# agwi-lab/renderformer

Measured on NVIDIA B200. Metric: frames/sec (512^2, 4096 tris), higher is better.
Workload: dtype bf16

## Files before the change

include/rfb200.h:

```cpp
#ifndef RFB200_H_
#define RFB200_H_

#include <stdint.h>

#ifdef __cplusplus
extern "C" {
#endif

typedef void* rfb_stream_t;

enum {
  RFB_OK = 0,
  RFB_ERR_ARG = -1,
  RFB_ERR_ALIGN = -2,
  RFB_ERR_DRIVER = -3,
  RFB_ERR_TMAP = -4,
  RFB_ERR_LAUNCH = -5
};

enum { RFB_F32 = 0, RFB_BF16 = 1, RFB_F16 = 2 };

int rfb_version(void);
long long rfb_launch_count(void);

// ... 38 lines not shown
  float norm_eps;
  float* out_rscale;
  float* out_sumsq;
  int out_sumsq_ld;
  void* out16;
  int out16_dtype;
  long long ld16;
  const float* col_mul;
  const int* aux_row_map;
  void* vt_out;
  int vt_dtype;
  int vt_split;
  int vt_rows_per_batch;
  long long vt_ld;
  long long vt_batch_stride;
} rfb_gemm_args;

int rfb_gemm(const rfb_gemm_args* a, rfb_stream_t stream);

typedef struct {
  int B, H, Nq, Nk;
  const void* Q;
  long long ldq, q_batch_stride;
  const void* K;
  long long ldk, k_batch_stride;
  const void* Vt;
  long long ldvt, vt_batch_stride;
  void* O;
  long long ldo, o_batch_stride;
  const uint32_t* key_mask_bits;
// ... 79 lines not shown
```

renderformer_b200/csrc/gemm.cu:

```cuda
#include <stdlib.h>

#include <atomic>

#include "host_util.h"
#include "ptx.cuh"

namespace rfb {

std::atomic<long long> g_launch_count{0};

struct GemmKParams {
  int M, N, K;
  int num_m_tiles, num_n_tiles, num_kb;
  int a_mode;
  int H, Wd, Cin, tw, th, tiles_x, tiles_y, kb_per_tap;
  uint32_t idesc;
  int epi;
  const float* bias;
  const void* res1;
  const void* res2;
  int res_dtype;
  long long ldres;
  void* out;
  int out_dtype;
// ... 731 lines not shown
      if (cudaFuncGetAttributes(&fa, gemm_tc_kernel<BN, EK>) != cudaSuccess) return RFB_ERR_LAUNCH;
      if (128 * kRegsGemmWg0 + 256 * kRegsGemmEpi > kGemmThreadsWG * fa.numRegs) {
        fprintf(stderr, "rfb: gemm_tc_kernel<RESID> compiled with %d registers/thread; setmaxnreg split does not fit\n",
                fa.numRegs);
        return RFB_ERR_LAUNCH;
      }
    }
    attr_set = true;
  }
  constexpr int threads = ek_resid(EK) ? kGemmThreadsWG : kGemmThreads;
  gemm_tc_kernel<BN, EK><<<grid, threads, Cfg::kSmemBytes, stream>>>(tmA, tmB, p);
  g_launch_count++;
  return check_launch("gemm_tc_kernel");
}

constexpr int kHaloPitch = 18;
constexpr uint32_t kHaloBytes = kHaloPitch * kHaloPitch * 128;
constexpr uint32_t kHaloStride = 42 * 1024;

template <int BN>
struct HaloCfg {
  static constexpr uint32_t kBBytes = BN * kBK * 2;
  static constexpr int kStages = (BN == 128) ? 6 : 8;
  static constexpr uint32_t kTmemCols = (4 * BN < 32) ? 32 : 4 * BN;
  static constexpr uint32_t kSmemBytes = 2 * kHaloStride + kStages * kBBytes + 1024 + 256 + kEpiStageBytes;
};

template <int BN, int EK>
__global__ void __launch_bounds__(kGemmThreads, 1)
    conv_halo_kernel(const __grid_constant__ CUtensorMap tmA, const __grid_constant__ CUtensorMap tmB,
                     const GemmKParams p) {
  using Cfg = HaloCfg<BN>;
  constexpr int STAGES = Cfg::kStages;
  constexpr uint32_t B_BYTES = Cfg::kBBytes;

  extern __shared__ uint8_t smem_raw[];
  const uint32_t raw_addr = smem_u32(smem_raw);
  uint8_t* smem = smem_raw + ((1024u - (raw_addr & 1023u)) & 1023u);
  uint8_t* sH = smem;
  uint8_t* sB = smem + 2 * kHaloStride;
  uint64_t* bfull = reinterpret_cast<uint64_t*>(sB + STAGES * B_BYTES);
  uint64_t* bempty = bfull + STAGES;
  uint64_t* hfull = bempty + STAGES;
  uint64_t* hempty = hfull + 2;
  uint64_t* tfull = hempty + 2;
  uint64_t* tempty = tfull + 2;
  uint32_t* tmem_slot = reinterpret_cast<uint32_t*>(tempty + 2);
  float* epi_stage = reinterpret_cast<float*>(reinterpret_cast<uint8_t*>(bfull) + 256);

  const int warp = threadIdx.x >> 5;
  const int lane = threadIdx.x & 31;

  if (threadIdx.x == 0) {
    for (int i = 0; i < STAGES; ++i) mbar_init(&bfull[i], 1), mbar_init(&bempty[i], 1);
    for (int i = 0; i < 2; ++i) {
// ... 11 lines not shown
  tc_fence_before();
  __syncthreads();
  tc_fence_after();
  const uint32_t tmem_base = *tmem_slot;

  const int per_img = p.tiles_x * p.tiles_y;
  const int total = p.num_m_tiles;
  const int ncb = p.kb_per_tap;

  if (warp == 0) {
    if (lane == 0) {
      int stage = 0, hb = 0;
      uint32_t phase = 0, hphase = 0;
      for (int tile = blockIdx.x; tile < total; tile += gridDim.x) {
        const int bi = tile / per_img, rr = tile % per_img;
        const int y0 = (rr / p.tiles_x) * 16, x0 = (rr % p.tiles_x) * 16;
        for (int cb = 0; cb < ncb; ++cb) {
          mbar_wait(&hempty[hb], hphase ^ 1);
          mbar_expect_tx(&hfull[hb], kHaloBytes);
          tma_load_4d(sH + hb * kHaloStride, &tmA, &hfull[hb], cb * kBK, x0 - 1, y0 - 1, bi);
          if (++hb == 2) hb = 0, hphase ^= 1;
          for (int tap = 0; tap < 9; ++tap) {
            mbar_wait(&bempty[stage], phase ^ 1);
            mbar_expect_tx(&bfull[stage], B_BYTES);
            tma_load_2d(sB + stage * B_BYTES, &tmB, &bfull[stage], tap * p.Cin + cb * kBK, 0);
            if (++stage == STAGES) stage = 0, phase ^= 1;
          }
        }
      }
    }
  } else if (warp == 1) {
    if (lane == 0) {
      int stage = 0, hb = 0, it = 0;
      uint32_t phase = 0, hphase = 0;
      for (int tile = blockIdx.x; tile < total; tile += gridDim.x, ++it) {
        const int as = it & 1;
        mbar_wait(&tempty[as], ((it >> 1) & 1) ^ 1);
        tc_fence_after();
        const uint32_t d0 = tmem_base + as * 2 * BN;
        for (int cb = 0; cb < ncb; ++cb) {
          mbar_wait(&hfull[hb], hphase);
          tc_fence_after();
          const uint32_t halo = smem_u32(sH + hb * kHaloStride);
          for (int tap = 0; tap < 9; ++tap) {
            mbar_wait(&bfull[stage], phase);
            tc_fence_after();
            const uint64_t bd = umma_desc_sw128(smem_u32(sB + stage * B_BYTES));
            const uint32_t a0 = halo + ((tap / 3) * kHaloPitch + tap % 3) * 128;
#pragma unroll
            for (int t = 0; t < 2; ++t) {
              uint64_t ad = static_cast<uint64_t>(((a0 + t * 8 * 128) >> 4) & 0x3fff);
              ad |= static_cast<uint64_t>((kHaloPitch * 128) >> 4) << 32;
              ad |= static_cast<uint64_t>(1) << 46;
              ad |= static_cast<uint64_t>(2) << 61;
#pragma unroll
              for (int k = 0; k < kBK / 16; ++k)
                umma_f16(d0 + t * BN, ad + 2 * k, bd + 2 * k, p.idesc, (cb | tap | k) != 0);
            }
            umma_commit(&bempty[stage]);
            if (++stage == STAGES) stage = 0, phase ^= 1;
          }
          umma_commit(&hempty[hb]);
          if (++hb == 2) hb = 0, hphase ^= 1;
        }
        umma_commit(&tfull[as]);
      }
    }
  } else {
    const int q = warp & 3;
    const int r = q * 32 + lane;
    int it = 0;
    for (int tile = blockIdx.x; tile < total; tile += gridDim.x, ++it) {
      const int as = it & 1;
      const uint32_t aph = (it >> 1) & 1;
      const int bi = tile / per_img, rr = tile % per_img;
      const int y = (rr / p.tiles_x) * 16 + (r >> 3);
      float* my_stage = epi_stage + (warp - 2) * 32 * 32;
      constexpr int NCH = BN / 32;
      constexpr int HALF = (NCH + 1) / 2;
      const int c_begin = ((warp - 2) >> 2) * HALF;
      const int c_end = (c_begin + HALF < NCH) ? c_begin + HALF : NCH;
#pragma unroll 1
      for (int t = 0; t < 2; ++t) {
        const int x = (rr % p.tiles_x) * 16 + t * 8 + (r & 7);
        const bool valid = (y < p.H) && (x < p.Wd);
        const long long orow = (static_cast<long long>(bi) * p.H + y) * p.Wd + x;
        const int orow_mine = valid ? static_cast<int>(orow) : -1;
        const uint32_t taddr0 = tmem_base + (static_cast<uint32_t>(q * 32) << 16) + as * 2 * BN + t * BN;
        if (p.epi == RFB_EPI_STORE) {
          epilogue_generic_coalesced<EK>(p, my_stage, lane, taddr0, 0, c_begin, c_end, orow_mine, orow_mine, 1.0f,
                                         &tfull[as], aph);
        } else {
// ... 11 lines not shown
      }
      tc_fence_before();
      __syncwarp();
      if (lane == 0) mbar_arrive(&tempty[as]);
    }
  }

  tc_fence_before();
  __syncthreads();
  if (warp == 1) {
    tc_fence_after();
    tmem_dealloc(tmem_base, Cfg::kTmemCols);
  }
}

template <int BN, int EK = EK_GENERIC>
static int launch_conv_halo(const CUtensorMap& tmA, const CUtensorMap& tmB, const GemmKParams& p, int grid,
                            cudaStream_t stream) {
  using Cfg = HaloCfg<BN>;
  static PerDeviceFlag attr_flags;
  bool& attr_set = attr_flags.get();
  if (!attr_set) {
    if (cudaFuncSetAttribute(conv_halo_kernel<BN, EK>, cudaFuncAttributeMaxDynamicSharedMemorySize,
                             Cfg::kSmemBytes) != cudaSuccess)
      return RFB_ERR_LAUNCH;
    attr_set = true;
  }
  conv_halo_kernel<BN, EK><<<grid, kGemmThreads, Cfg::kSmemBytes, stream>>>(tmA, tmB, p);
  g_launch_count++;
  return check_launch("conv_halo_kernel");
}

}

using namespace rfb;

extern "C" int rfb_gemm(const rfb_gemm_args* a, rfb_stream_t stream_) {
  cudaStream_t stream = static_cast<cudaStream_t>(stream_);
  if (!a || !a->A || !a->W || a->M <= 0 || a->N <= 0 || a->K <= 0) return RFB_ERR_ARG;
  if (a->dtype != RFB_BF16 && a->dtype != RFB_F16) return RFB_ERR_ARG;

  GemmKParams p{};
  p.M = a->M, p.N = a->N, p.K = a->K;
// ... 7 lines not shown
  p.in_sumsq_parts = a->in_sumsq_parts > 0 ? a->in_sumsq_parts : 1;
  p.in_rscale = a->in_rscale, p.scale_dim = a->scale_dim, p.out_rscale = a->out_rscale;
  p.inv_norm_dim = a->norm_dim > 0 ? 1.0f / (float)a->norm_dim : 0.f;
  p.norm_eps = a->norm_eps;
  p.out_sumsq = a->out_sumsq, p.out_sumsq_ld = a->out_sumsq_ld;
  p.out16 = a->out16, p.out16_dtype = a->out16_dtype, p.ld16 = a->ld16;
  p.col_mul = a->col_mul, p.aux_row_map = a->aux_row_map;
  p.vt_out = a->vt_out, p.vt_dtype = a->vt_dtype, p.vt_split = a->vt_split;
  p.vt_rows_per_batch = a->vt_rows_per_batch, p.vt_ld = a->vt_ld, p.vt_batch_stride = a->vt_batch_stride;
  if (a->vt_out) {
    if (a->a_mode != RFB_A_LINEAR || a->epi != RFB_EPI_STORE || a->row_map || a->vt_split <= 0 || a->vt_split >= a->N ||
        a->vt_split % 256 || (a->vt_dtype != RFB_BF16 && a->vt_dtype != RFB_F16) || a->vt_ld < 1 ||
        (a->in_rscale && a->scale_dim == 1))
      return RFB_ERR_ARG;
  }
  const bool fused_any = a->in_sumsq || a->in_rscale || a->out_rscale || a->out_sumsq || a->out16 || a->col_mul;
  if (a->in_sumsq && (a->norm_dim <= 0 || a->in_rscale || p.in_sumsq_parts > p.in_sumsq_ld)) return RFB_ERR_ARG;
  if (a->in_rscale && a->scale_dim != 0 && a->scale_dim != 1) return RFB_ERR_ARG;
  if (a->out_rscale && !a->in_sumsq) return RFB_ERR_ARG;
  const bool epi_final = a->epi == RFB_EPI_FINAL || a->epi == RFB_EPI_FINAL_RAW;
  if (fused_any && epi_final) return RFB_ERR_ARG;
  if (a->epi == RFB_EPI_SWIGLU && (a->out_rscale || a->out_sumsq || a->out16 || a->col_mul ||
                                   (a->in_rscale && a->scale_dim != 0)))
    return RFB_ERR_ARG;
  if (a->out16 && (a->ld16 % 8 || (a->out16_dtype != RFB_BF16 && a->out16_dtype != RFB_F16))) return RFB_ERR_ARG;
  if (a->out16 && a->N % 8) return RFB_ERR_ARG;
  const int n_plain = a->vt_out ? a->vt_split : a->N;
  if (a->out_sumsq && (n_plain % 128 || a->out_sumsq_ld < n_plain / 128)) return RFB_ERR_ARG;
  if (a->res2 && (a->res_dtype == RFB_F32 || !a->res1)) return RFB_ERR_ARG;

  const bool resid_kind = a->epi == RFB_EPI_STORE && a->a_mode == RFB_A_LINEAR && a->N % 256 == 0 && a->out16 &&
                          a->out_sumsq && !a->bias && !a->res2 && !a->out_act && !a->vt_out && !a->col_mul &&
                          !(a->in_rscale && a->scale_dim == 1) && a->out && a->out_dtype == RFB_F32 && a->res1 &&
                          a->res_dtype == RFB_F32;
  const int sms = num_sms();
  const long long m_tiles_lin = (a->M + kBM - 1) / kBM;
  int bn = a->bn_override;
  if (a->vt_out) {
    if (bn != 0 && bn != 256) return RFB_ERR_ARG;
    bn = 256;
  }
  if (a->out_sumsq) {
// ... 18 lines not shown
  }
  if (bn != 32 && bn != 64 && bn != 128 && bn != 256) return RFB_ERR_ARG;

  if (a->epi == RFB_EPI_STORE) {
    p.n_store = (n_plain + 7) & ~7;
    if (p.n_store > a->ldo) return RFB_ERR_ARG;
    if ((a->bias || a->res1 || a->res2) && (a->N % 8) != 0) return RFB_ERR_ARG;
    if (!a->out && !a->out_act && !a->out16) return RFB_ERR_ARG;
    const int align = (a->out_dtype == RFB_F32) ? 4 : 8;
    if (a->ldo % align) return RFB_ERR_ALIGN;
    if ((a->res1 || a->res2) && a->ldres % ((a->res_dtype == RFB_F32) ? 4 : 8)) return RFB_ERR_ALIGN;
  } else if (a->epi == RFB_EPI_SWIGLU) {
    if (a->N % 32 || !a->out || a->out_dtype == RFB_F32 || a->ldo % 8) return RFB_ERR_ARG;
    p.n_store = a->N;
  } else if (epi_final) {
    if (a->N != 32 || !a->out || !a->bias || !a->w2 || !a->b2) return RFB_ERR_ARG;
    bn = 32;
    p.n_store = 32;
  } else {
    return RFB_ERR_ARG;
  }

  CUtensorMap tmA, tmB;
  int rc;
  if (a->a_mode == RFB_A_LINEAR) {
    uint64_t dims[2] = {(uint64_t)a->K, (uint64_t)a->M};
    uint64_t strides[1] = {(uint64_t)a->lda * 2};
    uint32_t box[2] = {(uint32_t)kBK, (uint32_t)kBM};
    if ((rc = make_tmap_16b(&tmA, a->dtype, a->A, 2, dims, strides, box)) != RFB_OK) return rc;
    p.num_m_tiles = (a->M + kBM - 1) / kBM;
    p.num_kb = (a->K + kBK - 1) / kBK;
  } else if (a->a_mode == RFB_A_CONV3X3) {
    if (a->B <= 0 || a->H <= 0 || a->Wd <= 0 || a->Cin <= 0 || a->K != 9 * a->Cin ||
        a->M != a->B * a->H * a->Wd || a->row_map)
      return RFB_ERR_ARG;
    {
      static int halo_on = -1;
      if (halo_on < 0) {
        const char* e = getenv("RFB_CONV_HALO");
        halo_on = (e && e[0] == '0') ? 0 : 1;
      }
      const int stx = (a->Wd + 15) / 16, sty = (a->H + 15) / 16;
      const long long n_super = (long long)a->B * stx * sty;
      if (halo_on && a->Cin % 64 == 0 && a->N == bn && (bn == 128 || bn == 64 || bn == 32) && n_super >= 96 &&
          !fused_any && !a->vt_out && !p.direct_store) {
        p.H = a->H, p.Wd = a->Wd, p.Cin = a->Cin;
        p.tw = 8, p.th = 16, p.tiles_x = stx, p.tiles_y = sty, p.kb_per_tap = a->Cin / kBK;
        p.num_m_tiles = (int)n_super, p.num_n_tiles = 1, p.num_kb = 9 * p.kb_per_tap;
        uint64_t dims[4] = {(uint64_t)a->Cin, (uint64_t)a->Wd, (uint64_t)a->H, (uint64_t)a->B};
        uint64_t strides[3] = {(uint64_t)a->Cin * 2, (uint64_t)a->Wd * a->Cin * 2, (uint64_t)a->H * a->Wd * a->Cin * 2};
        uint32_t box[4] = {(uint32_t)kBK, (uint32_t)kHaloPitch, (uint32_t)kHaloPitch, 1};
        if ((rc = make_tmap_16b(&tmA, a->dtype, a->A, 4, dims, strides, box)) != RFB_OK) return rc;
        uint64_t wd[2] = {(uint64_t)a->K, (uint64_t)a->N};
        uint64_t ws[1] = {(uint64_t)a->ldw * 2};
        uint32_t wb[2] = {(uint32_t)kBK, (uint32_t)bn};
        if ((rc = make_tmap_16b(&tmB, a->dtype, a->W, 2, wd, ws, wb)) != RFB_OK) return rc;
        p.idesc = umma_idesc_f16(a->dtype == RFB_BF16 ? 1u : 0u, kBM, bn);
        const int cap = a->max_ctas > 0 ? a->max_ctas : num_sms();
        const int grid = (int)(n_super < cap ? n_super : cap);
        if (bn == 64) return launch_conv_halo<64>(tmA, tmB, p, grid, stream);
        if (bn == 32) return launch_conv_halo<32>(tmA, tmB, p, grid, stream);
        if (a->epi == RFB_EPI_STORE && a->dtype == RFB_F16 && a->out_dtype == RFB_F16 &&
            (!a->res1 || a->res_dtype == RFB_F16)) {
          const int cm = (a->out ? CF_OUT : 0) | (a->out_act ? CF_ACT : 0) | (a->bias ? CF_BIAS : 0) |
                         (a->res1 ? CF_RES1 : 0) | (a->res2 ? CF_RES2 : 0);
          switch (cm) {
// ... 55 lines not shown
  if (bn == 128 && a->out_sumsq) {
    if (p.direct_store) return RFB_ERR_ARG;
    return a->out16_dtype == RFB_F16 ? launch_gemm<128, EK_RESID_H>(tmA, tmB, p, grid, stream)
                                     : launch_gemm<128, EK_RESID>(tmA, tmB, p, grid, stream);
  }
  if (bn == 256 && a->N % 256 == 0 && a->epi == RFB_EPI_STORE && !p.direct_store && a->out16 &&
      a->out_sumsq && !a->bias && !a->res2 && !a->out_act && !(a->in_rscale && a->scale_dim == 1)) {
    const bool half = a->out16_dtype == RFB_F16;
    if (a->out && a->out_dtype == RFB_F32 && a->res1 && a->res_dtype == RFB_F32 && !a->col_mul)
      return half ? launch_gemm<256, EK_RESID_H>(tmA, tmB, p, grid, stream)
                  : launch_gemm<256, EK_RESID>(tmA, tmB, p, grid, stream);
    if (!a->out && !a->res1 && a->col_mul)
      return half ? launch_gemm<256, EK_PROJ16_H>(tmA, tmB, p, grid, stream)
                  : launch_gemm<256, EK_PROJ16>(tmA, tmB, p, grid, stream);
  }
  if (bn == 128 && a->a_mode == RFB_A_CONV3X3 && a->epi == RFB_EPI_STORE && !p.direct_store && !fused_any && !a->vt_out &&
      a->dtype == RFB_F16 && a->out_dtype == RFB_F16 && (!a->res1 || a->res_dtype == RFB_F16) && a->N % 128 == 0) {
    const int cm = (a->out ? CF_OUT : 0) | (a->out_act ? CF_ACT : 0) | (a->bias ? CF_BIAS : 0) | (a->res1 ? CF_RES1 : 0) |
                   (a->res2 ? CF_RES2 : 0);
    switch (cm) {
      case CF_OUT | CF_ACT: return launch_gemm<128, EK_CONV + (CF_OUT | CF_ACT)>(tmA, tmB, p, grid, stream);
      case CF_ACT | CF_BIAS: return launch_gemm<128, EK_CONV + (CF_ACT | CF_BIAS)>(tmA, tmB, p, grid, stream);
      case CF_OUT | CF_BIAS | CF_RES1:
        return launch_gemm<128, EK_CONV + (CF_OUT | CF_BIAS | CF_RES1)>(tmA, tmB, p, grid, stream);
      case CF_OUT | CF_ACT | CF_BIAS | CF_RES1:
        return launch_gemm<128, EK_CONV + (CF_OUT | CF_ACT | CF_BIAS | CF_RES1)>(tmA, tmB, p, grid, stream);
      case CF_OUT | CF_BIAS | CF_RES1 | CF_RES2:
        return launch_gemm<128, EK_CONV + (CF_OUT | CF_BIAS | CF_RES1 | CF_RES2)>(tmA, tmB, p, grid, stream);
      case CF_OUT | CF_ACT | CF_BIAS | CF_RES1 | CF_RES2:
        return launch_gemm<128, EK_CONV + (CF_OUT | CF_ACT | CF_BIAS | CF_RES1 | CF_RES2)>(tmA, tmB, p, grid, stream);
      default: break;
    }
  }
  switch (bn) {
    case 32: return launch_gemm<32>(tmA, tmB, p, grid, stream);
// ... 9 lines not shown
```

renderformer_b200/engine.py:

```python
from __future__ import annotations

from dataclasses import dataclass
from typing import Callable, Dict, List, Optional

import torch

from . import lib as L
from . import ops
from .config import RenderFormerConfig

EPS = 1e-6


def _rup(x: int, m: int) -> int:
    return (x + m - 1) // m * m


@dataclass
class SceneState:
    B: int
    N: int
    Nt: int
    Ntp: int
    seq: torch.Tensor
# ... 37 lines not shown


def swin_window_maps(Hp: int, Wp: int, shift: int, ws: int = 8):
    w = torch.arange(Hp * Wp)
    win, p = w // (ws * ws), w % (ws * ws)
    ry = (win // (Wp // ws)) * ws + p // ws
    rx = (win % (Wp // ws)) * ws + p % ws
    perm = ((ry + shift) % Hp) * Wp + (rx + shift) % Wp
    if shift > 0:
        def rid(r, n):
            return (r >= n - ws).long() + (r >= n - shift).long()
        region = 3 * rid(ry, Hp) + rid(rx, Wp)
    else:
        region = torch.zeros_like(w)
    return perm.to(torch.int32), region.to(torch.uint8)


ALL_PARTS = ("tokens", "ray", "encoder", "decoder", "dpt")


class Engine:
    def __init__(self, cfg: RenderFormerConfig, state_dict: Dict[str, torch.Tensor], device, parts=ALL_PARTS,
                 op_dtype: torch.dtype = torch.bfloat16):
        cfg.check_supported()
        if op_dtype not in (torch.bfloat16, torch.float16):
            raise ValueError("op_dtype must be torch.bfloat16 or torch.float16")
        self.cfg = cfg
        self.op = op_dtype
        self.parts = tuple(parts)
        self.device = torch.device(device)
        if self.device.type != "cuda":
            raise L.RfbError("renderformer_b200.Engine needs a CUDA device (there is no CPU fallback)")
        L.load()
        self.fused_dec = bool(cfg.view_transformer_use_swin_attn)
        self.w: Dict[str, torch.Tensor] = {}
        self._maps: Dict[tuple, tuple] = {}
        self._prepare(state_dict)

    def _prepare(self, sd: Dict[str, torch.Tensor]) -> None:
        cfg, dev = self.cfg, self.device
        bf, hf = self.op, torch.float16

        def g(k):
            return sd[k].detach().to(dev, torch.float32)

        def put(name, t, dt=None):
            self.w[name] = (t if dt is None else t.to(dt)).contiguous()

        def swiglu_w(p):
# ... 103 lines not shown
            put(f"dpt.rn{i}.w", conv_w(h + f"scratch.layer{i + 1}_rn.weight"), hf)
        for i, s in ((0, 4), (1, 2)):
            w = g(h + f"resize_layers.{i}.weight")
            put(f"dpt.up{i}.w", w.permute(2, 3, 1, 0).reshape(s * s * w.shape[1], w.shape[0]), hf)
            put(f"dpt.up{i}.b", g(h + f"resize_layers.{i}.bias").repeat(s * s))
        put("dpt.down3.w", conv_w(h + "resize_layers.3.weight"), hf), put("dpt.down3.b", g(h + "resize_layers.3.bias"))
        for r in (1, 2, 3, 4):
            p = h + f"scratch.refinenet{r}."
            put(f"dpt.rf{r}.out.w", g(p + "out_conv.weight").flatten(1), hf), put(f"dpt.rf{r}.out.b", g(p + "out_conv.bias"))
            for u in ((1, 2) if r != 4 else (2,)):
                for c in (1, 2):
                    put(f"dpt.rf{r}.u{u}c{c}.w", conv_w(p + f"resConvUnit{u}.conv{c}.weight"), hf)
                    put(f"dpt.rf{r}.u{u}c{c}.b", g(p + f"resConvUnit{u}.conv{c}.bias"))
        put("dpt.oc1.w", conv_w(h + "scratch.output_conv1.weight"), hf), put("dpt.oc1.b", g(h + "scratch.output_conv1.bias"))
        put("dpt.oc2.w", conv_w(h + "scratch.output_conv2.0.weight"), hf), put("dpt.oc2.b", g(h + "scratch.output_conv2.0.bias"))
        put("dpt.oc3.w", g(h + "scratch.output_conv2.2.weight").flatten(1)), put("dpt.oc3.b", g(h + "scratch.output_conv2.2.bias"))

    def _e(self, shape, dtype):
        return torch.empty(shape, dtype=dtype, device=self.device)

    def _ffn(self, x, rows, d, n_w, w13, w2):
        h = ops.rmsnorm(x, n_w, self._e((rows, d), self.op), rows=rows, d=d, eps=EPS)
        g = ops.gemm(h, w13, epi=L.EPI_SWIGLU, out_dtype=self.op)
        ops.gemm(g, w2, out=x, res1=x)

    @torch.no_grad()
    def encode_scene(self, triangles, texture, mask, vn, texture_is_log: bool = False,
                     shard: Optional[RowShard] = None, texture_own_rows: bool = False,
                     taps: Optional[dict] = None, gather_seq: bool = False) -> SceneState:
        cfg, w, dev = self.cfg, self.w, self.device
# ... 370 lines not shown
        for i in range(cfg.view_transformer_n_layers):
            o = f"dec{i}."
            perm, region, inv = self._swin_maps(Hp, Wp, 0 if i % 2 == 0 else 4, V)
            ops.gemm(xb, w[o + "wq"], out16=qh, col_mul=w[o + "qn"], out_sumsq=qsq, in_sumsq=xsq, **nrm)
            ops.attention(qh, kall[:, i * dv:], st.v_t(i, b), att, B=V, H=Hh, Nq=Nr, Nk=Ntp, ldq=dv, ldk=Lv * dv,
                          ldvt=Ntp, ldo=dv, q_bs=Nr * dv, k_bs=Ntp * Lv * dv, vt_bs=0, o_bs=Nr * dv,
                          mask_bits=st.mask_bits[b], mask_bs=0, q_sumsq=qsq, sumsq_ld=P, sumsq_parts=P, **nrm)
            ops.gemm(att, w[o + "wout"], out=x, res1=x, out_sumsq=xsqw, out16=xbw, aux_row_map=inv)
            ops.gemm(xbw, w[o + "s.wqkv"], out16=qkh, col_mul=w[o + "s.qkn"], out_sumsq=qksq, in_sumsq=xsqw,
                     vt_out=vt, vt_split=2 * dv, **nrm)
            ops.attention(qkh, qkh[:, dv:], vt, att, B=1, H=Hh, Nq=rows, Nk=rows, ldq=2 * dv, ldk=2 * dv,
                          ldvt=rows, ldo=dv, mode=1, group_id=region, group_period=Nr,
                          q_sumsq=qksq, k_sumsq=qksq.view(-1)[P:], sumsq_ld=2 * P, sumsq_parts=P, **nrm)
            ops.gemm(att, w[o + "s.wo"], out=x, res1=x, row_map=perm, out_sumsq=xsq, out16=xb)
            g = ops.gemm(xb, w[o + "w13"], epi=L.EPI_SWIGLU, out_dtype=bf, in_sumsq=xsq, **nrm)
            ops.gemm(g, w[o + "w2"], out=x, res1=x, out_sumsq=xsq, out16=xb)
            if i in out_layers:
                feats.append(x.clone() if want_f32 else ops.cast(x, self._e((rows, dv), torch.float16)))
                if taps is not None:
                    taps.setdefault("dec_feats", []).append(x.clone().view(V, Nr, dv))
        return feats

    def _conv(self, x, name, B, H, W, Cin, **kw):
        return ops.gemm(x, self.w[name + ".w"], conv=(B, H, W, Cin), **kw)

    def _rcu(self, x_raw, x_act, name, B, H, W, extra_res=None, want_act=False):
        F_ = self.cfg.dpt_features
        hf = torch.float16
        t = self._e((B * H * W, F_), hf)
        self._conv(x_act, name + "c1", B, H, W, F_, bias=self.w[name + "c1.b"], out=None, out_act=t)
        out = self._e((B * H * W, F_), hf)
        act = self._e((B * H * W, F_), hf) if want_act else None
        self._conv(t, name + "c2", B, H, W, F_, bias=self.w[name + "c2.b"], res1=x_raw, res2=extra_res, out=out,
                   out_act=act)
        return out, act

    def _fusion(self, r, B, H, W, Ho, Wo, x0, x1_raw=None, x1_act=None, x0_act=None):
        F_ = self.cfg.dpt_features
        hf = torch.float16
# ... 2 lines not shown
            s_raw, s_act = self._rcu(x1_raw, x1_act, name + "u1", B, H, W, extra_res=x0, want_act=True)
        else:
            s_raw, s_act = x0, x0_act
        o, _ = self._rcu(s_raw, s_act, name + "u2", B, H, W)
        o = ops.gemm(o, self.w[name + "out.w"], bias=self.w[name + "out.b"], out=self._e((B * H * W, F_), hf))
        return ops.upsample_bilinear(o, self._e((B * Ho * Wo, F_), hf), B=B, Hi=H, Wi=W, Ho=Ho, Wo=Wo, C_=F_)

    def _dpt(self, feats, V, Hp, Wp, raw_out: bool = False, out: Optional[torch.Tensor] = None):
        cfg, w = self.cfg, self.w
        hf = torch.float16
        C = list(cfg.dpt_out_channels)
        F_ = cfg.dpt_features
        n = V * Hp * Wp
        proj = [ops.gemm(feats[i], w[f"dpt.proj{i}.w"], bias=w[f"dpt.proj{i}.b"], out=self._e((n, C[i]), hf))
                for i in range(4)]
        t0 = ops.gemm(proj[0], w["dpt.up0.w"], bias=w["dpt.up0.b"], out=self._e((n, 16 * C[0]), hf))
        r0 = ops.pixel_shuffle(t0, self._e((V * 16 * Hp * Wp, C[0]), hf), B=V, h=Hp, w=Wp, s=4, C_=C[0])
        t1 = ops.gemm(proj[1], w["dpt.up1.w"], bias=w["dpt.up1.b"], out=self._e((n, 4 * C[1]), hf))
        r1 = ops.pixel_shuffle(t1, self._e((V * 4 * Hp * Wp, C[1]), hf), B=V, h=Hp, w=Wp, s=2, C_=C[1])
        r2 = proj[2]
        H3, W3 = (Hp + 1) // 2, (Wp + 1) // 2
        col = ops.im2col_s2(proj[3], self._e((V * H3 * W3, 9 * C[3]), hf), B=V, H=Hp, W=Wp, C_=C[3])
        r3 = ops.gemm(col, w["dpt.down3.w"], bias=w["dpt.down3.b"], out=self._e((V * H3 * W3, C[3]), hf))
        dims = [(4 * Hp, 4 * Wp), (2 * Hp, 2 * Wp), (Hp, Wp), (H3, W3)]
        lraw, lact = [], []
        for i, (r, (H, W)) in enumerate(zip((r0, r1, r2, r3), dims)):
            raw, act = self._e((V * H * W, F_), hf), self._e((V * H * W, F_), hf)
            self._conv(r, f"dpt.rn{i}", V, H, W, C[i], out=raw, out_act=act)
            lraw.append(raw), lact.append(act)
        p4 = self._fusion(4, V, *dims[3], *dims[2], lraw[3], x0_act=lact[3])
        p3 = self._fusion(3, V, *dims[2], *dims[1], p4, lraw[2], lact[2])
        p2 = self._fusion(2, V, *dims[1], *dims[0], p3, lraw[1], lact[1])
        Ho, Wo = 8 * Hp, 8 * Wp
        p1 = self._fusion(1, V, *dims[0], Ho, Wo, p2, lraw[0], lact[0])
        o1 = self._conv(p1, "dpt.oc1", V, Ho, Wo, F_, bias=w["dpt.oc1.b"], out=self._e((V * Ho * Wo, F_ // 2), hf))
        if out is not None and (tuple(out.shape) != (V, Ho, Wo, 3) or out.dtype != torch.float32 or not out.is_contiguous()):
            raise ValueError("out must be a contiguous fp32 [V, H, W, 3] tensor")
        img = out if out is not None else self._e((V, Ho, Wo, 3), torch.float32)
        self._conv(o1, "dpt.oc2", V, Ho, Wo, F_ // 2, bias=w["dpt.oc2.b"], epi=L.EPI_FINAL_RAW if raw_out else L.EPI_FINAL,
                   w2=w["dpt.oc3.w"], b2=w["dpt.oc3.b"], out=img, ldo=3)
        return img
```

renderformer_b200/lib.py:

```python
from __future__ import annotations

import ctypes as C
import os

_HERE = os.path.dirname(os.path.abspath(__file__))
LIB_PATH = os.path.join(_HERE, "librfb200.so")

F32, BF16, F16 = 0, 1, 2
A_LINEAR, A_CONV3X3 = 0, 1
EPI_STORE, EPI_SWIGLU, EPI_FINAL, EPI_FINAL_RAW = 0, 1, 2, 3

_ERRORS = {-1: "bad argument / unsupported shape", -2: "misaligned pointer or stride",
           -3: "CUDA driver entry point unavailable", -4: "tensor map rejected", -5: "kernel launch failed"}


class RfbError(RuntimeError):
    pass


class GemmArgs(C.Structure):
    _fields_ = [
        ("M", C.c_int), ("N", C.c_int), ("K", C.c_int),
        ("A", C.c_void_p), ("lda", C.c_longlong),
        ("W", C.c_void_p), ("ldw", C.c_longlong),
# ... 1 lines not shown
        ("B", C.c_int), ("H", C.c_int), ("Wd", C.c_int), ("Cin", C.c_int),
        ("epi", C.c_int),
        ("bias", C.c_void_p), ("res1", C.c_void_p), ("res2", C.c_void_p),
        ("res_dtype", C.c_int), ("ldres", C.c_longlong),
        ("out", C.c_void_p), ("out_dtype", C.c_int), ("ldo", C.c_longlong),
        ("out_act", C.c_void_p), ("row_map", C.c_void_p),
        ("w2", C.c_void_p), ("b2", C.c_void_p),
        ("bn_override", C.c_int), ("max_ctas", C.c_int),
        ("in_sumsq", C.c_void_p), ("in_sumsq_ld", C.c_int), ("in_sumsq_parts", C.c_int),
        ("in_rscale", C.c_void_p), ("scale_dim", C.c_int), ("norm_dim", C.c_int), ("norm_eps", C.c_float),
        ("out_rscale", C.c_void_p), ("out_sumsq", C.c_void_p), ("out_sumsq_ld", C.c_int),
        ("out16", C.c_void_p), ("out16_dtype", C.c_int), ("ld16", C.c_longlong),
        ("col_mul", C.c_void_p), ("aux_row_map", C.c_void_p),
        ("vt_out", C.c_void_p), ("vt_dtype", C.c_int), ("vt_split", C.c_int), ("vt_rows_per_batch", C.c_int),
        ("vt_ld", C.c_longlong), ("vt_batch_stride", C.c_longlong),
    ]


class AttnArgs(C.Structure):
    _fields_ = [
        ("B", C.c_int), ("H", C.c_int), ("Nq", C.c_int), ("Nk", C.c_int),
        ("Q", C.c_void_p), ("ldq", C.c_longlong), ("q_batch_stride", C.c_longlong),
        ("K", C.c_void_p), ("ldk", C.c_longlong), ("k_batch_stride", C.c_longlong),
        ("Vt", C.c_void_p), ("ldvt", C.c_longlong), ("vt_batch_stride", C.c_longlong),
        ("O", C.c_void_p), ("ldo", C.c_longlong), ("o_batch_stride", C.c_longlong),
        ("key_mask_bits", C.c_void_p), ("mask_batch_stride_words", C.c_longlong),
        ("mode", C.c_int), ("group_id", C.c_void_p), ("group_period", C.c_int),
        ("scale", C.c_float),
        ("q_sumsq", C.c_void_p), ("k_sumsq", C.c_void_p), ("sumsq_ld", C.c_int), ("sumsq_parts", C.c_int),
        ("norm_dim", C.c_int),
# ... 68 lines not shown
```

renderformer_b200/ops.py:

```python
from __future__ import annotations

import ctypes as C
from typing import Optional

import torch

from . import lib as L

_DT = {torch.float32: L.F32, torch.bfloat16: L.BF16, torch.float16: L.F16}


PROFILE = None


_DEV = [None]


def _timed(kind: str, flops: float, launch, tag: str = ""):
    dev = _DEV[0]
    if dev is not None and dev.index is not None and dev.index != torch.cuda.current_device():
        with torch.cuda.device(dev):
            return _timed_on_device(kind, flops, launch, tag)
    return _timed_on_device(kind, flops, launch, tag)

# ... 23 lines not shown
        if t is None:
            continue
        if not t.is_cuda:
            raise L.RfbError("renderformer_b200 kernels need CUDA tensors (there is no CPU fallback)")
        if dev is None:
            dev = t.device
        elif t.device != dev:
            raise L.RfbError(f"operands live on different devices ({dev} vs {t.device})")
    _DEV[0] = dev


def gemm(A: torch.Tensor, W: torch.Tensor, out: Optional[torch.Tensor] = None, *, M=None, N=None, K=None,
         bias=None, res1=None, res2=None, out_act=None, row_map=None, epi=L.EPI_STORE, out_dtype=None,
         conv=None, w2=None, b2=None, lda=None, ldw=None, ldo=None, ldres=None, bn=0,
         in_sumsq=None, in_rscale=None, scale_dim=0, norm_dim=0, norm_eps=1e-6, out_rscale=None, out_sumsq=None,
         out16=None, col_mul=None, aux_row_map=None, vt_out=None, vt_split=0, vt_rows_per_batch=0) -> torch.Tensor:
    _need_cuda(A, W)
    lib = L.load()
    a = L.GemmArgs()
    if conv is not None:
        Bc, Hc, Wc, Cin = conv
        a.a_mode, a.B, a.H, a.Wd, a.Cin = L.A_CONV3X3, Bc, Hc, Wc, Cin
        M = Bc * Hc * Wc if M is None else M
        K = 9 * Cin if K is None else K
        lda = Cin
    else:
        M = A.shape[0] if M is None else M
        K = A.shape[-1] if K is None else K
        lda = A.stride(0) if lda is None else lda
    N = W.shape[0] if N is None else N
    ldw = W.stride(0) if ldw is None else ldw
    a.M, a.N, a.K, a.A, a.lda, a.W, a.ldw = M, N, K, A.data_ptr(), lda, W.data_ptr(), ldw
    a.dtype = _DT[A.dtype]
    assert W.dtype == A.dtype, "operand dtypes differ"
    a.epi = epi
    if out is None and out_act is None and out16 is None:
        ncols = N // 2 if epi == L.EPI_SWIGLU else (3 if epi in (L.EPI_FINAL, L.EPI_FINAL_RAW) else N)
        out = torch.empty((M, ncols), dtype=out_dtype or torch.float32, device=A.device)
    ref = out if out is not None else out_act
    a.out, a.out_act = _p(out), _p(out_act)
    if ref is not None:
        a.out_dtype = _DT[ref.dtype]
        a.ldo = (ref.stride(0) if ref.dim() == 2 else ref.shape[-1]) if ldo is None else ldo
    else:
        a.out_dtype, a.ldo = L.F32, _rup8(N)
    if in_sumsq is not None:
        a.in_sumsq, a.in_sumsq_ld, a.in_sumsq_parts = in_sumsq.data_ptr(), in_sumsq.stride(0), in_sumsq.shape[1]
        a.norm_dim, a.norm_eps = norm_dim, norm_eps
    if in_rscale is not None:
        a.in_rscale, a.scale_dim = in_rscale.data_ptr(), scale_dim
    a.out_rscale = _p(out_rscale)
    if out_sumsq is not None:
# ... 4 lines not shown
    if vt_out is not None:
        a.vt_out, a.vt_dtype, a.vt_split = vt_out.data_ptr(), _DT[vt_out.dtype], vt_split
        a.vt_ld = vt_out.stride(-2)
        a.vt_rows_per_batch = vt_rows_per_batch
        a.vt_batch_stride = vt_out.stride(0) if vt_out.dim() == 3 else 0
    a.bias = _p(bias)
    if res1 is not None:
        a.res1, a.res_dtype = res1.data_ptr(), _DT[res1.dtype]
        a.ldres = (res1.stride(0) if res1.dim() == 2 else res1.shape[-1]) if ldres is None else ldres
    if res2 is not None:
        a.res2 = res2.data_ptr()
    a.row_map = _p(row_map)
    a.w2, a.b2 = _p(w2), _p(b2)
    a.bn_override = bn
    tag = f"M={M} N={N} K={K} epi={epi} conv={int(conv is not None)} out={a.out_dtype} res={int(res1 is not None)}"
    L.check(_timed("gemm", 2.0 * M * N * K, lambda: lib.rfb_gemm(C.byref(a), _stream()), tag), "rfb_gemm")
    return out if out is not None else (out_act if out_act is not None else out16)


def _rup8(n: int) -> int:
    return (n + 7) // 8 * 8


def attention(Q, K, Vt, O, *, B, H, Nq, Nk, ldq, ldk, ldvt, ldo, q_bs=0, k_bs=0, vt_bs=0, o_bs=0,
              mask_bits=None, mask_bs=0, mode=0, group_id=None, group_period=0, scale=None,
              q_sumsq=None, k_sumsq=None, sumsq_ld=1, sumsq_parts=1, norm_dim=0, norm_eps=1e-6,
              kv_split_tiles=0, split_ws=None):
    _need_cuda(Q, K, Vt, O)
    lib = L.load()
    a = L.AttnArgs()
    if kv_split_tiles > 0 and attention_ws_elems(B, H, Nq, Nk, kv_split_tiles) > 0:
# ... 178 lines not shown
```

Baseline: 290.7.

## Pack two output rows per conv halo tile and fuse conv-transpose shuffle

Adds an R=2 halo conv kernel that covers two output rows per tile. Weights are packed so the two row outputs become a single 2*Co wide GEMM over 12 taps. This is used for the DPT output convs to raise MMA N width and halo reuse, at the cost of extra zero-padded weight FLOPs. Separately, the conv-transpose upsample plus pixel_shuffle is replaced by row-mapped GEMM stores, the last decoder tap is written straight to fp16, and a new bias-only fp16 fast-path kernel variant is added.

```diff
diff --git a/include/rfb200.h b/include/rfb200.h
--- a/include/rfb200.h
+++ b/include/rfb200.h
@@ -76,6 +76,7 @@
   int vt_rows_per_batch;
   long long vt_ld;
   long long vt_batch_stride;
+  int conv_rows;
 } rfb_gemm_args;
 
 int rfb_gemm(const rfb_gemm_args* a, rfb_stream_t stream);
diff --git a/renderformer_b200/csrc/gemm.cu b/renderformer_b200/csrc/gemm.cu
--- a/renderformer_b200/csrc/gemm.cu
+++ b/renderformer_b200/csrc/gemm.cu
@@ -769,23 +769,36 @@
   return check_launch("gemm_tc_kernel");
 }
 
-constexpr int kHaloPitch = 18;
-constexpr uint32_t kHaloBytes = kHaloPitch * kHaloPitch * 128;
-constexpr uint32_t kHaloStride = 42 * 1024;
-
-template <int BN>
+template <int R>
+struct HaloGeom {
+  static constexpr int kW = 18;
+  static constexpr int kH = 16 * R + 2;
+  static constexpr int kTiles = 2;
+  static constexpr int kTileW = 16;
+  static constexpr int kTileH = 16 * R;
+  static constexpr int kTaps = (R + 2) * 3;
+  static constexpr uint32_t kBytes = kW * kH * 128;
+  static constexpr uint32_t kStride = R == 1 ? 42 * 1024 : (kBytes + 1023) / 1024 * 1024;
+  static constexpr uint32_t kSbo = R * kW * 128;
+};
+static_assert(HaloGeom<1>::kTaps == 9 && HaloGeom<2>::kTaps == 12, "tap counts");
+
+template <int BN, int R>
 struct HaloCfg {
   static constexpr uint32_t kBBytes = BN * kBK * 2;
-  static constexpr int kStages = (BN == 128) ? 6 : 8;
+  static constexpr int kStages = (BN == 128) ? (R == 1 ? 6 : 4) : 8;
   static constexpr uint32_t kTmemCols = (4 * BN < 32) ? 32 : 4 * BN;
-  static constexpr uint32_t kSmemBytes = 2 * kHaloStride + kStages * kBBytes + 1024 + 256 + kEpiStageBytes;
+  static constexpr uint32_t kSmemBytes =
+      2 * HaloGeom<R>::kStride + kStages * kBBytes + 1024 + 256 + (R == 1 ? kEpiStageBytes : 0);
+  static_assert(kSmemBytes <= 227 * 1024, "halo kernel shared memory");
 };
 
-template <int BN, int EK>
+template <int BN, int EK, int R>
 __global__ void __launch_bounds__(kGemmThreads, 1)
     conv_halo_kernel(const __grid_constant__ CUtensorMap tmA, const __grid_constant__ CUtensorMap tmB,
                      const GemmKParams p) {
-  using Cfg = HaloCfg<BN>;
+  using Cfg = HaloCfg<BN, R>;
+  using G = HaloGeom<R>;
   constexpr int STAGES = Cfg::kStages;
   constexpr uint32_t B_BYTES = Cfg::kBBytes;
 
@@ -793,7 +806,7 @@
   const uint32_t raw_addr = smem_u32(smem_raw);
   uint8_t* smem = smem_raw + ((1024u - (raw_addr & 1023u)) & 1023u);
   uint8_t* sH = smem;
-  uint8_t* sB = smem + 2 * kHaloStride;
+  uint8_t* sB = smem + 2 * G::kStride;
   uint64_t* bfull = reinterpret_cast<uint64_t*>(sB + STAGES * B_BYTES);
   uint64_t* bempty = bfull + STAGES;
   uint64_t* hfull = bempty + STAGES;
@@ -835,13 +848,13 @@
       uint32_t phase = 0, hphase = 0;
       for (int tile = blockIdx.x; tile < total; tile += gridDim.x) {
         const int bi = tile / per_img, rr = tile % per_img;
-        const int y0 = (rr / p.tiles_x) * 16, x0 = (rr % p.tiles_x) * 16;
+        const int y0 = (rr / p.tiles_x) * G::kTileH, x0 = (rr % p.tiles_x) * G::kTileW;
         for (int cb = 0; cb < ncb; ++cb) {
           mbar_wait(&hempty[hb], hphase ^ 1);
-          mbar_expect_tx(&hfull[hb], kHaloBytes);
-          tma_load_4d(sH + hb * kHaloStride, &tmA, &hfull[hb], cb * kBK, x0 - 1, y0 - 1, bi);
+          mbar_expect_tx(&hfull[hb], G::kBytes);
+          tma_load_4d(sH + hb * G::kStride, &tmA, &hfull[hb], cb * kBK, x0 - 1, y0 - 1, bi);
           if (++hb == 2) hb = 0, hphase ^= 1;
-          for (int tap = 0; tap < 9; ++tap) {
+          for (int tap = 0; tap < G::kTaps; ++tap) {
             mbar_wait(&bempty[stage], phase ^ 1);
             mbar_expect_tx(&bfull[stage], B_BYTES);
             tma_load_2d(sB + stage * B_BYTES, &tmB, &bfull[stage], tap * p.Cin + cb * kBK, 0);
@@ -858,20 +871,20 @@
         const int as = it & 1;
         mbar_wait(&tempty[as], ((it >> 1) & 1) ^ 1);
         tc_fence_after();
-        const uint32_t d0 = tmem_base + as * 2 * BN;
+        const uint32_t d0 = tmem_base + as * G::kTiles * BN;
         for (int cb = 0; cb < ncb; ++cb) {
           mbar_wait(&hfull[hb], hphase);
           tc_fence_after();
-          const uint32_t halo = smem_u32(sH + hb * kHaloStride);
-          for (int tap = 0; tap < 9; ++tap) {
+          const uint32_t halo = smem_u32(sH + hb * G::kStride);
+          for (int tap = 0; tap < G::kTaps; ++tap) {
             mbar_wait(&bfull[stage], phase);
             tc_fence_after();
             const uint64_t bd = umma_desc_sw128(smem_u32(sB + stage * B_BYTES));
-            const uint32_t a0 = halo + ((tap / 3) * kHaloPitch + tap % 3) * 128;
-#pragma unroll
-            for (int t = 0; t < 2; ++t) {
+            const uint32_t a0 = halo + ((tap / 3) * G::kW + tap % 3) * 128;
+#pragma unroll
+            for (int t = 0; t < G::kTiles; ++t) {
               uint64_t ad = static_cast<uint64_t>(((a0 + t * 8 * 128) >> 4) & 0x3fff);
-              ad |= static_cast<uint64_t>((kHaloPitch * 128) >> 4) << 32;
+              ad |= static_cast<uint64_t>(G::kSbo >> 4) << 32;
               ad |= static_cast<uint64_t>(1) << 46;
               ad |= static_cast<uint64_t>(2) << 61;
 #pragma unroll
@@ -895,8 +908,33 @@
       const int as = it & 1;
       const uint32_t aph = (it >> 1) & 1;
       const int bi = tile / per_img, rr = tile % per_img;
+      float* my_stage = epi_stage + (warp - 2) * 32 * 32;
+      if constexpr (R == 2) {
+        const int half = (warp - 2) >> 2;
+        const int y = (rr / p.tiles_x) * G::kTileH + 2 * (r >> 3) + half;
+        mbar_wait(&tfull[as], aph);
+        tc_fence_after();
+#pragma unroll 1
+        for (int t = 0; t < 2; ++t) {
+          const int x = (rr % p.tiles_x) * G::kTileW + t * 8 + (r & 7);
+          const bool valid = (y < p.H) && (x < p.Wd);
+          const long long orow = (static_cast<long long>(bi) * p.H + y) * p.Wd + x;
+          const uint32_t taddr0 =
+              tmem_base + (static_cast<uint32_t>(q * 32) << 16) + (as * 2 + t) * BN + half * (BN / 2);
+#pragma unroll 1
+          for (int c = 0; c < BN / 64; ++c) {
+            uint32_t v[32];
+            tmem_ld32(taddr0 + c * 32, v);
+            tmem_wait_ld();
+            if (valid) epilogue_chunk(p, orow, c * 32, v, 1.0f);
+          }
+        }
+        tc_fence_before();
+        __syncwarp();
+        if (lane == 0) mbar_arrive(&tempty[as]);
+        continue;
+      }
       const int y = (rr / p.tiles_x) * 16 + (r >> 3);
-      float* my_stage = epi_stage + (warp - 2) * 32 * 32;
       constexpr int NCH = BN / 32;
       constexpr int HALF = (NCH + 1) / 2;
       const int c_begin = ((warp - 2) >> 2) * HALF;
@@ -938,19 +976,19 @@
   }
 }
 
-template <int BN, int EK = EK_GENERIC>
+template <int BN, int EK = EK_GENERIC, int R = 1>
 static int launch_conv_halo(const CUtensorMap& tmA, const CUtensorMap& tmB, const GemmKParams& p, int grid,
                             cudaStream_t stream) {
-  using Cfg = HaloCfg<BN>;
+  using Cfg = HaloCfg<BN, R>;
   static PerDeviceFlag attr_flags;
   bool& attr_set = attr_flags.get();
   if (!attr_set) {
-    if (cudaFuncSetAttribute(conv_halo_kernel<BN, EK>, cudaFuncAttributeMaxDynamicSharedMemorySize,
+    if (cudaFuncSetAttribute(conv_halo_kernel<BN, EK, R>, cudaFuncAttributeMaxDynamicSharedMemorySize,
                              Cfg::kSmemBytes) != cudaSuccess)
       return RFB_ERR_LAUNCH;
     attr_set = true;
   }
-  conv_halo_kernel<BN, EK><<<grid, kGemmThreads, Cfg::kSmemBytes, stream>>>(tmA, tmB, p);
+  conv_halo_kernel<BN, EK, R><<<grid, kGemmThreads, Cfg::kSmemBytes, stream>>>(tmA, tmB, p);
   g_launch_count++;
   return check_launch("conv_halo_kernel");
 }
@@ -988,6 +1026,8 @@
         (a->in_rscale && a->scale_dim == 1))
       return RFB_ERR_ARG;
   }
+  const int rows = a->conv_rows > 0 ? a->conv_rows : 1;
+  if (rows != 1 && rows != 2) return RFB_ERR_ARG;
   const bool fused_any = a->in_sumsq || a->in_rscale || a->out_rscale || a->out_sumsq || a->out16 || a->col_mul;
   if (a->in_sumsq && (a->norm_dim <= 0 || a->in_rscale || p.in_sumsq_parts > p.in_sumsq_ld)) return RFB_ERR_ARG;
   if (a->in_rscale && a->scale_dim != 0 && a->scale_dim != 1) return RFB_ERR_ARG;
@@ -999,7 +1039,7 @@
     return RFB_ERR_ARG;
   if (a->out16 && (a->ld16 % 8 || (a->out16_dtype != RFB_BF16 && a->out16_dtype != RFB_F16))) return RFB_ERR_ARG;
   if (a->out16 && a->N % 8) return RFB_ERR_ARG;
-  const int n_plain = a->vt_out ? a->vt_split : a->N;
+  const int n_plain = a->vt_out ? a->vt_split : a->N / rows;
   if (a->out_sumsq && (n_plain % 128 || a->out_sumsq_ld < n_plain / 128)) return RFB_ERR_ARG;
   if (a->res2 && (a->res_dtype == RFB_F32 || !a->res1)) return RFB_ERR_ARG;
 
@@ -1048,8 +1088,8 @@
     if (a->N % 32 || !a->out || a->out_dtype == RFB_F32 || a->ldo % 8) return RFB_ERR_ARG;
     p.n_store = a->N;
   } else if (epi_final) {
-    if (a->N != 32 || !a->out || !a->bias || !a->w2 || !a->b2) return RFB_ERR_ARG;
-    bn = 32;
+    if (a->N != 32 * rows || !a->out || !a->bias || !a->w2 || !a->b2) return RFB_ERR_ARG;
+    bn = a->N;
     p.n_store = 32;
   } else {
     return RFB_ERR_ARG;
@@ -1065,9 +1105,32 @@
     p.num_m_tiles = (a->M + kBM - 1) / kBM;
     p.num_kb = (a->K + kBK - 1) / kBK;
   } else if (a->a_mode == RFB_A_CONV3X3) {
-    if (a->B <= 0 || a->H <= 0 || a->Wd <= 0 || a->Cin <= 0 || a->K != 9 * a->Cin ||
+    if (a->B <= 0 || a->H <= 0 || a->Wd <= 0 || a->Cin <= 0 || a->K != (rows + 2) * 3 * a->Cin ||
         a->M != a->B * a->H * a->Wd || a->row_map)
       return RFB_ERR_ARG;
+    if (rows == 2) {
+      if (a->Cin % 64 || (a->N != 64 && a->N != 128) || bn != a->N || fused_any || a->vt_out || a->res2 ||
+          a->epi == RFB_EPI_SWIGLU || (a->epi == RFB_EPI_STORE && (a->out_act || a->res1)))
+        return RFB_ERR_ARG;
+      using G = HaloGeom<2>;
+      const int stx = (a->Wd + G::kTileW - 1) / G::kTileW, sty = (a->H + G::kTileH - 1) / G::kTileH;
+      p.H = a->H, p.Wd = a->Wd, p.Cin = a->Cin;
+      p.tiles_x = stx, p.tiles_y = sty, p.kb_per_tap = a->Cin / kBK;
+      p.num_m_tiles = a->B * stx * sty, p.num_n_tiles = 1, p.num_kb = G::kTaps * p.kb_per_tap;
+      uint64_t dims[4] = {(uint64_t)a->Cin, (uint64_t)a->Wd, (uint64_t)a->H, (uint64_t)a->B};
+      uint64_t strides[3] = {(uint64_t)a->Cin * 2, (uint64_t)a->Wd * a->Cin * 2, (uint64_t)a->H * a->Wd * a->Cin * 2};
+      uint32_t box[4] = {(uint32_t)kBK, (uint32_t)G::kW, (uint32_t)G::kH, 1};
+      if ((rc = make_tmap_16b(&tmA, a->dtype, a->A, 4, dims, strides, box)) != RFB_OK) return rc;
+      uint64_t wd[2] = {(uint64_t)a->K, (uint64_t)a->N};
+      uint64_t ws[1] = {(uint64_t)a->ldw * 2};
+      uint32_t wb[2] = {(uint32_t)kBK, (uint32_t)bn};
+      if ((rc = make_tmap_16b(&tmB, a->dtype, a->W, 2, wd, ws, wb)) != RFB_OK) return rc;
+      p.idesc = umma_idesc_f16(a->dtype == RFB_BF16 ? 1u : 0u, kBM, bn);
+      const int cap = a->max_ctas > 0 ? a->max_ctas : num_sms();
+      const int grid = p.num_m_tiles < cap ? p.num_m_tiles : cap;
+      if (bn == 64) return launch_conv_halo<64, EK_GENERIC, 2>(tmA, tmB, p, grid, stream);
+      return launch_conv_halo<128, EK_GENERIC, 2>(tmA, tmB, p, grid, stream);
+    }
     {
       static int halo_on = -1;
       if (halo_on < 0) {
@@ -1083,7 +1146,7 @@
         p.num_m_tiles = (int)n_super, p.num_n_tiles = 1, p.num_kb = 9 * p.kb_per_tap;
         uint64_t dims[4] = {(uint64_t)a->Cin, (uint64_t)a->Wd, (uint64_t)a->H, (uint64_t)a->B};
         uint64_t strides[3] = {(uint64_t)a->Cin * 2, (uint64_t)a->Wd * a->Cin * 2, (uint64_t)a->H * a->Wd * a->Cin * 2};
-        uint32_t box[4] = {(uint32_t)kBK, (uint32_t)kHaloPitch, (uint32_t)kHaloPitch, 1};
+        uint32_t box[4] = {(uint32_t)kBK, (uint32_t)HaloGeom<1>::kW, (uint32_t)HaloGeom<1>::kH, 1};
         if ((rc = make_tmap_16b(&tmA, a->dtype, a->A, 4, dims, strides, box)) != RFB_OK) return rc;
         uint64_t wd[2] = {(uint64_t)a->K, (uint64_t)a->N};
         uint64_t ws[1] = {(uint64_t)a->ldw * 2};
@@ -1169,11 +1232,12 @@
       return half ? launch_gemm<256, EK_PROJ16_H>(tmA, tmB, p, grid, stream)
                   : launch_gemm<256, EK_PROJ16>(tmA, tmB, p, grid, stream);
   }
-  if (bn == 128 && a->a_mode == RFB_A_CONV3X3 && a->epi == RFB_EPI_STORE && !p.direct_store && !fused_any && !a->vt_out &&
+  if (bn == 128 && a->epi == RFB_EPI_STORE && !p.direct_store && !fused_any && !a->vt_out &&
       a->dtype == RFB_F16 && a->out_dtype == RFB_F16 && (!a->res1 || a->res_dtype == RFB_F16) && a->N % 128 == 0) {
     const int cm = (a->out ? CF_OUT : 0) | (a->out_act ? CF_ACT : 0) | (a->bias ? CF_BIAS : 0) | (a->res1 ? CF_RES1 : 0) |
                    (a->res2 ? CF_RES2 : 0);
     switch (cm) {
+      case CF_OUT | CF_BIAS: return launch_gemm<128, EK_CONV + (CF_OUT | CF_BIAS)>(tmA, tmB, p, grid, stream);
       case CF_OUT | CF_ACT: return launch_gemm<128, EK_CONV + (CF_OUT | CF_ACT)>(tmA, tmB, p, grid, stream);
       case CF_ACT | CF_BIAS: return launch_gemm<128, EK_CONV + (CF_ACT | CF_BIAS)>(tmA, tmB, p, grid, stream);
       case CF_OUT | CF_BIAS | CF_RES1:
diff --git a/renderformer_b200/engine.py b/renderformer_b200/engine.py
--- a/renderformer_b200/engine.py
+++ b/renderformer_b200/engine.py
@@ -75,6 +75,16 @@
     else:
         region = torch.zeros_like(w)
     return perm.to(torch.int32), region.to(torch.uint8)
+
+
+def pack_conv_rows(w: torch.Tensor, rows: int = 2) -> torch.Tensor:
+    Co, K9 = w.shape
+    Cin = K9 // 9
+    w4 = w.reshape(Co, 3, 3, Cin)
+    out = w.new_zeros(rows, Co, rows + 2, 3, Cin)
+    for j in range(rows):
+        out[j, :, j:j + 3] = w4
+    return out.reshape(rows * Co, (rows + 2) * 3 * Cin)
 
 
 ALL_PARTS = ("tokens", "ray", "encoder", "decoder", "dpt")
@@ -94,6 +104,7 @@
             raise L.RfbError("renderformer_b200.Engine needs a CUDA device (there is no CPU fallback)")
         L.load()
         self.fused_dec = bool(cfg.view_transformer_use_swin_attn)
+        self.dpt_packed = True
         self.w: Dict[str, torch.Tensor] = {}
         self._maps: Dict[tuple, tuple] = {}
         self._prepare(state_dict)
@@ -227,6 +238,8 @@
                     put(f"dpt.rf{r}.u{u}c{c}.b", g(p + f"resConvUnit{u}.conv{c}.bias"))
         put("dpt.oc1.w", conv_w(h + "scratch.output_conv1.weight"), hf), put("dpt.oc1.b", g(h + "scratch.output_conv1.bias"))
         put("dpt.oc2.w", conv_w(h + "scratch.output_conv2.0.weight"), hf), put("dpt.oc2.b", g(h + "scratch.output_conv2.0.bias"))
+        for n in ("oc1", "oc2"):
+            put(f"dpt.{n}.w2rows", pack_conv_rows(self.w[f"dpt.{n}.w"]))
         put("dpt.oc3.w", g(h + "scratch.output_conv2.2.weight").flatten(1)), put("dpt.oc3.b", g(h + "scratch.output_conv2.2.bias"))
 
     def _e(self, shape, dtype):
@@ -627,15 +640,35 @@
                           q_sumsq=qksq, k_sumsq=qksq.view(-1)[P:], sumsq_ld=2 * P, sumsq_parts=P, **nrm)
             ops.gemm(att, w[o + "s.wo"], out=x, res1=x, row_map=perm, out_sumsq=xsq, out16=xb)
             g = ops.gemm(xb, w[o + "w13"], epi=L.EPI_SWIGLU, out_dtype=bf, in_sumsq=xsq, **nrm)
-            ops.gemm(g, w[o + "w2"], out=x, res1=x, out_sumsq=xsq, out16=xb)
+            tap16 = self._e((rows, dv), torch.float16) if i == Lv - 1 and i in out_layers and not want_f32 else None
+            ops.gemm(g, w[o + "w2"], out=x, res1=x, out_sumsq=xsq, out16=xb if tap16 is None else tap16)
             if i in out_layers:
-                feats.append(x.clone() if want_f32 else ops.cast(x, self._e((rows, dv), torch.float16)))
+                if tap16 is not None:
+                    feats.append(tap16)
+                else:
+                    feats.append(x.clone() if want_f32 else ops.cast(x, self._e((rows, dv), torch.float16)))
                 if taps is not None:
                     taps.setdefault("dec_feats", []).append(x.clone().view(V, Nr, dv))
         return feats
 
-    def _conv(self, x, name, B, H, W, Cin, **kw):
-        return ops.gemm(x, self.w[name + ".w"], conv=(B, H, W, Cin), **kw)
+    def _conv_transpose(self, x, name, V, Hp, Wp, s, Co):
+        key = ("shuffle", V, Hp, Wp, s)
+        if key not in self._maps:
+            b, h, w_ = torch.meshgrid(torch.arange(V), torch.arange(Hp), torch.arange(Wp), indexing="ij")
+            self._maps[key] = ((b * s * Hp + s * h) * Wp + w_).reshape(-1).to(torch.int32).to(self.device).contiguous()
+        rmap = self._maps[key]
+        out = self._e((V * s * Hp * s * Wp, Co), torch.float16)
+        flat = out.view(-1)
+        wt, bias = self.w[name + ".w"], self.w[name + ".b"]
+        n = s * Co
+        for i in range(s):
+            ops.gemm(x, wt[i * n:(i + 1) * n], bias=bias[i * n:(i + 1) * n], out=flat[i * s * Wp * Co:], ldo=n,
+                     row_map=rmap)
+        return out
+
+    def _conv(self, x, name, B, H, W, Cin, rows=1, **kw):
+        w = self.w[name + (".w" if rows == 1 else f".w{rows}rows")]
+        return ops.gemm(x, w, conv=(B, H, W, Cin), conv_rows=rows, **kw)
 
     def _rcu(self, x_raw, x_act, name, B, H, W, extra_res=None, want_act=False):
         F_ = self.cfg.dpt_features
@@ -668,10 +701,8 @@
         n = V * Hp * Wp
         proj = [ops.gemm(feats[i], w[f"dpt.proj{i}.w"], bias=w[f"dpt.proj{i}.b"], out=self._e((n, C[i]), hf))
                 for i in range(4)]
-        t0 = ops.gemm(proj[0], w["dpt.up0.w"], bias=w["dpt.up0.b"], out=self._e((n, 16 * C[0]), hf))
-        r0 = ops.pixel_shuffle(t0, self._e((V * 16 * Hp * Wp, C[0]), hf), B=V, h=Hp, w=Wp, s=4, C_=C[0])
-        t1 = ops.gemm(proj[1], w["dpt.up1.w"], bias=w["dpt.up1.b"], out=self._e((n, 4 * C[1]), hf))
-        r1 = ops.pixel_shuffle(t1, self._e((V * 4 * Hp * Wp, C[1]), hf), B=V, h=Hp, w=Wp, s=2, C_=C[1])
+        r0 = self._conv_transpose(proj[0], "dpt.up0", V, Hp, Wp, 4, C[0])
+        r1 = self._conv_transpose(proj[1], "dpt.up1", V, Hp, Wp, 2, C[1])
         r2 = proj[2]
         H3, W3 = (Hp + 1) // 2, (Wp + 1) // 2
         col = ops.im2col_s2(proj[3], self._e((V * H3 * W3, 9 * C[3]), hf), B=V, H=Hp, W=Wp, C_=C[3])
@@ -687,10 +718,12 @@
         p2 = self._fusion(2, V, *dims[1], *dims[0], p3, lraw[1], lact[1])
         Ho, Wo = 8 * Hp, 8 * Wp
         p1 = self._fusion(1, V, *dims[0], Ho, Wo, p2, lraw[0], lact[0])
-        o1 = self._conv(p1, "dpt.oc1", V, Ho, Wo, F_, bias=w["dpt.oc1.b"], out=self._e((V * Ho * Wo, F_ // 2), hf))
+        rows = 2 if self.dpt_packed and F_ == 128 else 1
+        o1 = self._conv(p1, "dpt.oc1", V, Ho, Wo, F_, rows=rows, bias=w["dpt.oc1.b"],
+                        out=self._e((V * Ho * Wo, F_ // 2), hf))
         if out is not None and (tuple(out.shape) != (V, Ho, Wo, 3) or out.dtype != torch.float32 or not out.is_contiguous()):
             raise ValueError("out must be a contiguous fp32 [V, H, W, 3] tensor")
         img = out if out is not None else self._e((V, Ho, Wo, 3), torch.float32)
-        self._conv(o1, "dpt.oc2", V, Ho, Wo, F_ // 2, bias=w["dpt.oc2.b"], epi=L.EPI_FINAL_RAW if raw_out else L.EPI_FINAL,
+        self._conv(o1, "dpt.oc2", V, Ho, Wo, F_ // 2, rows=rows, bias=w["dpt.oc2.b"], epi=L.EPI_FINAL_RAW if raw_out else L.EPI_FINAL,
                    w2=w["dpt.oc3.w"], b2=w["dpt.oc3.b"], out=img, ldo=3)
         return img
diff --git a/renderformer_b200/lib.py b/renderformer_b200/lib.py
--- a/renderformer_b200/lib.py
+++ b/renderformer_b200/lib.py
@@ -39,6 +39,7 @@
         ("col_mul", C.c_void_p), ("aux_row_map", C.c_void_p),
         ("vt_out", C.c_void_p), ("vt_dtype", C.c_int), ("vt_split", C.c_int), ("vt_rows_per_batch", C.c_int),
         ("vt_ld", C.c_longlong), ("vt_batch_stride", C.c_longlong),
+        ("conv_rows", C.c_int),
     ]
 
 
diff --git a/renderformer_b200/ops.py b/renderformer_b200/ops.py
--- a/renderformer_b200/ops.py
+++ b/renderformer_b200/ops.py
@@ -61,15 +61,17 @@
          bias=None, res1=None, res2=None, out_act=None, row_map=None, epi=L.EPI_STORE, out_dtype=None,
          conv=None, w2=None, b2=None, lda=None, ldw=None, ldo=None, ldres=None, bn=0,
          in_sumsq=None, in_rscale=None, scale_dim=0, norm_dim=0, norm_eps=1e-6, out_rscale=None, out_sumsq=None,
-         out16=None, col_mul=None, aux_row_map=None, vt_out=None, vt_split=0, vt_rows_per_batch=0) -> torch.Tensor:
+         out16=None, col_mul=None, aux_row_map=None, vt_out=None, vt_split=0, vt_rows_per_batch=0,
+         conv_rows=1) -> torch.Tensor:
     _need_cuda(A, W)
     lib = L.load()
     a = L.GemmArgs()
     if conv is not None:
         Bc, Hc, Wc, Cin = conv
         a.a_mode, a.B, a.H, a.Wd, a.Cin = L.A_CONV3X3, Bc, Hc, Wc, Cin
+        a.conv_rows = conv_rows
         M = Bc * Hc * Wc if M is None else M
-        K = 9 * Cin if K is None else K
+        K = (conv_rows + 2) * 3 * Cin if K is None else K
         lda = Cin
     else:
         M = A.shape[0] if M is None else M
@@ -82,7 +84,7 @@
     assert W.dtype == A.dtype, "operand dtypes differ"
     a.epi = epi
     if out is None and out_act is None and out16 is None:
-        ncols = N // 2 if epi == L.EPI_SWIGLU else (3 if epi in (L.EPI_FINAL, L.EPI_FINAL_RAW) else N)
+        ncols = N // 2 if epi == L.EPI_SWIGLU else (3 if epi in (L.EPI_FINAL, L.EPI_FINAL_RAW) else N // conv_rows)
         out = torch.empty((M, ncols), dtype=out_dtype or torch.float32, device=A.device)
     ref = out if out is not None else out_act
     a.out, a.out_act = _p(out), _p(out_act)
@@ -117,7 +119,11 @@
     a.w2, a.b2 = _p(w2), _p(b2)
     a.bn_override = bn
     tag = f"M={M} N={N} K={K} epi={epi} conv={int(conv is not None)} out={a.out_dtype} res={int(res1 is not None)}"
-    L.check(_timed("gemm", 2.0 * M * N * K, lambda: lib.rfb_gemm(C.byref(a), _stream()), tag), "rfb_gemm")
+    flops = 2.0 * M * N * K
+    if conv_rows > 1:
+        tag += f" rows={conv_rows}"
+        flops = 2.0 * M * (N // conv_rows) * 9 * conv[3]
+    L.check(_timed("gemm", flops, lambda: lib.rfb_gemm(C.byref(a), _stream()), tag), "rfb_gemm")
     return out if out is not None else (out_act if out_act is not None else out16)
 
 
```

New measurement: 293.4, median of 6. No clear change (+0.9%).
